# folkol/query-engines

Measured on AMD Instinct MI355X. Metric: rows/sec filter+project+group-by over 1B-row Arrow batch; % HBM roofline, higher is better.
Workload: dtype int64; 1 GPU; C4: SELECT k, SUM(a+b), COUNT(*), MIN(a), MAX(b) WHERE a > 2^19 GROUP BY k; rows_per_gpu=1000000000, groups=1024, columns=k, a, b int64 (Arrow, no nulls), parallelism=hash-sharded partial aggregate x1

## Files before the change

query-engines_amd/csrc/qe_dev.hpp:

```cpp
#ifndef QE_DEV_HPP
#define QE_DEV_HPP

#ifndef QE_OP_EQ
#define QE_OP_EQ 10
#define QE_OP_NE 11
#define QE_OP_LT 12
#define QE_OP_LE 13
#define QE_OP_GT 14
#define QE_OP_GE 15
#endif
#ifndef QE_MAX_KEYS
#define QE_MAX_KEYS 4
#define QE_MAX_AGGS 8
#define QE_MAX_COLS 8
#define QE_MAX_TERMS 8
#define QE_MAX_TOKENS 16
#endif
#ifndef QE_AGG_SUM
#define QE_AGG_SUM 1
#define QE_AGG_MIN 2
#define QE_AGG_MAX 3
#define QE_AGG_COUNT 4
#define QE_AGG_COUNT_STAR 5
#define QE_AGG_AVG 6
// ... 75 lines not shown
  qu64 cap;
  qu64* ctl;
};

struct Plan {
  DCol cols[QE_MAX_COLS];
  DTerm terms[QE_MAX_TERMS];
  DAgg aggs[QE_MAX_AGGS];
  DTable t;
  qi64 n, row_base;
  const qu32* defer_in;
  qu32* defer_out;
  qu8* ovf;
  qu64 ovf_cap;
  qi32 ncols, nterms, mask_col, naggs;
  qi32 key_mode, nkeys, key_f64, rec_bytes;
  qi32 key_col[QE_MAX_KEYS], key_shift[QE_MAX_KEYS], key_nullbit[QE_MAX_KEYS], pad0;
  qi64 key_fmask[QE_MAX_KEYS];
  qi32 lds_log2, off_cstar;
  qi32 all8;
  qi32 nn_skip;
  qi32 off_acc[QE_MAX_AGGS], off_nn[QE_MAX_AGGS], off_idx[QE_MAX_AGGS];
  qu8* part_rec;
  qi64* part_off;
  qi64 part_tw;
  qi64* part_slice;
  qi64* part_chunk;
  qi32* part_sorted;
  qi32 mp_n, mp_pass;
  qi32 part_narrow;
  qi32 lds_compact;
  qu64 mp_keep;
  qu64* host_ctl;
};

__host__ __device__ inline qi64 f64_bits(double d) { return __builtin_bit_cast(qi64, d); }
__host__ __device__ inline double bits_f64(qi64 b) { return __builtin_bit_cast(double, b); }

__host__ __device__ inline qi64 f64_okey(double d) {
  const qi64 b = f64_bits(d == 0.0 ? 0.0 : d);
  return b >= 0 ? b : (b ^ 0x7FFFFFFFFFFFFFFFll);
}
__host__ __device__ inline double okey_f64(qi64 k) { return bits_f64(k >= 0 ? k : (k ^ 0x7FFFFFFFFFFFFFFFll)); }

__host__ __device__ inline qu64 fmix64(qu64 k) {
  k ^= k >> 33;
  k *= 0xFF51AFD7ED558CCDull;
  k ^= k >> 33;
  k *= 0xC4CEB9FE1A85EC53ull;
  k ^= k >> 33;
  return k;
}

__device__ inline qu32 spill_hash(qu64 key) {
  qu32 x = (qu32)key ^ (qu32)(key >> 32) * 0x27D4EB2Fu;
  x ^= x >> 16;
  x *= 0x85EBCA6Bu;
  x ^= x >> 13;
  x *= 0xC2B2AE35u;
  return x ^ (x >> 16);
}

__device__ inline qu32 lds_hash(qu64 key) {
  const qu32 x = (qu32)key ^ (qu32)(key >> 32) * 0x85EBCA6Bu;
  return x * 0x9E3779B1u;
}
// ... 804 lines not shown
```

query-engines_amd/csrc/qe_hashagg.hip:

```cpp
#include <map>
#include <memory>
#include <mutex>

#include "qe_internal.hpp"

namespace qe {

constexpr int HA_THREADS = 512;

__device__ __forceinline__ qi64* lds_keys(char* smem) { return (qi64*)smem; }

__device__ __forceinline__ void lds_init(const Plan& P, char* smem) {
  const int SS = (1 << P.lds_log2) + 2;
  qi64* keys = lds_keys(smem);
  qu32* cst = (qu32*)(smem + P.off_cstar);
  for (int s = threadIdx.x; s < SS; s += blockDim.x) {
    keys[s] = EMPTY_KEY;
    cst[s] = 0;
  }
#pragma unroll
  for (int j = 0; j < QE_MAX_AGGS; ++j) {
    if (j >= P.naggs) break;
    const DAgg& a = P.aggs[j];
    if (a.acc != ACC_NONE) {
      qi64* acc = (qi64*)(smem + P.off_acc[j]);
      const qi64 id = acc_identity(a.acc);
      for (int s = threadIdx.x; s < SS; s += blockDim.x) acc[s] = id;
    }
    if (a.track_nn) {
      qu32* nn = (qu32*)(smem + P.off_nn[j]);
      for (int s = threadIdx.x; s < SS; s += blockDim.x) nn[s] = 0;
    }
// ... 1319 lines not shown
  int32_t lds_log2_min = 0;
  int64_t expected_groups = 0;
  int64_t create_groups = 0;
  int grid = 0;
  int64_t* part_cnt = nullptr;
  size_t part_cnt_bytes = 0;
  int64_t chunk_cap = 0;
  uint8_t* part_rec = nullptr;
  size_t part_rec_bytes = 0;
  int64_t* part_slc = nullptr;
  size_t part_slc_bytes = 0;
  bool part_wide = false;
  bool narrow_failed = false;
  bool compact_off = false;
  uint8_t* ovf = nullptr;
  uint64_t ovf_cap = 0;
  uint32_t* defer[2] = {nullptr, nullptr};
  size_t defer_words = 0;
  bool defer_dirty[2] = {false, false};
  bool ctl_rows_clean = false;
  hipEvent_t ev[2] = {nullptr, nullptr};
  double last_kernel_ms = 0.0;
  int last_launches = 0;
  int last_specialized = 0;
  uint64_t last_sig = 0;
  std::string jit_note;
  bool async = false;
  bool pending = false;
  std::unique_ptr<qe::Plan> pend_plan;
  size_t pend_lds = 0;
  int pend_out_i = 0;
  uint64_t* ctl_pin = nullptr;
  hipEvent_t ev_ctl = nullptr;
  int poisoned = 0;
  std::string poison_msg;
  qe::Keyed* keyed = nullptr;
  int32_t flags = 0;
  uint64_t version = 0;
};

namespace qe {

int hashagg_expected_groups(const qe_hashagg* h, int64_t* out) {
  QE_CHECK(h && out, QE_ERR_INVALID_ARG, "null argument");
  *out = h->create_groups;
  return QE_OK;
}

qe_ctx* hashagg_ctx(const qe_hashagg* h) { return h ? h->ctx : nullptr; }

HashaggInfo hashagg_info(const qe_hashagg* h) {
  HashaggInfo I{};
  I.ctx = h->ctx;
  I.km = h->km;
  I.rec_bytes = h->rec_bytes;
  I.naggs = h->naggs;
  I.flags = h->flags;
  for (int j = 0; j < h->naggs; ++j) I.aggs[j] = h->aggs[j];
  I.version = h->version;
  I.ctl = (uint64_t*)h->ctl;
  I.keyed = h->keyed;
  return I;
}

static AggMeta agg_meta(const qe_hashagg* h) {
  AggMeta m{};
// ... 3 lines not shown
    m.acc[j] = h->acc[j];
    m.any_x = m.any_x || h->acc[j] == ACC_SUM_X;
  }
  m.nn_implicit = h->nn_implicit;
  return m;
}

static int32_t all_nn_bits(const qe_hashagg* h) {
  if (!agg_knobs().nn_implicit) return 0;
  int32_t b = 0;
  for (int j = 0; j < h->naggs; ++j)
    if (h->aggs[j].fn != QE_AGG_COUNT_STAR) b |= 1 << j;
  return b;
}

static int nn_materialize(qe_hashagg* h, int32_t mask) {
  mask &= h->nn_implicit;
  if (!mask) return QE_OK;
  const int grid = (int)std::min<uint64_t>(div_up(h->t.cap + 2, 256), 4096);
  hipLaunchKernelGGL(k_nn_materialize, dim3(grid), dim3(256), 0, h->ctx->stream, h->t, (qi32)mask);
  QE_TRY(launch_check("k_nn_materialize"));
  h->nn_implicit &= ~mask;
  return QE_OK;
}

static size_t table_bytes(const qe_hashagg* h, uint64_t cap) {
  const uint64_t SS = cap + 2;
  size_t b = 16 * SS;
  for (int j = 0; j < h->naggs; ++j)
    b += (16 + (acc_has_idx(h->acc[j]) ? 32 : 0) + (h->acc[j] == ACC_SUM_X ? 8 * FXE_WORDS : 0)) * SS;
  return b;
}

static int table_alloc(qe_hashagg* h, uint64_t cap, void** mem, DTable* t, qu64* zero_ctl = nullptr) {
  const size_t bytes = table_bytes(h, cap);
  QE_TRY(dev_alloc(h->ctx, bytes, mem));
  const uint64_t SS = cap + 2;
  char* p = (char*)*mem;
  *t = DTable{};
  t->keys = (qi64*)p;
  p += 8 * SS;
  t->cstar = (qu64*)p;
  p += 8 * SS;
  for (int j = 0; j < h->naggs; ++j) {
    t->acc[j] = (qi64*)p;
    p += 8 * SS;
    t->nn[j] = (qu64*)p;
    p += 8 * SS;
    if (acc_has_idx(h->acc[j])) {
      t->idx[j] = (qu64*)p;
      p += 32 * SS;
    }
  }
  char* e0 = p;
  for (int j = 0; j < h->naggs; ++j)
    if (h->acc[j] == ACC_SUM_X) {
      t->ext[j] = (qu64*)p;
      p += 8 * FXE_WORDS * SS;
    }
  if (p > e0) QE_HIP(hipMemsetAsync(e0, 0, (size_t)(p - e0), h->ctx->stream));
  t->cap = cap;
  t->ctl = h->ctl;
  const int grid = (int)std::min<uint64_t>(div_up(SS, 256), 4096);
  hipLaunchKernelGGL(k_table_init, dim3(grid), dim3(256), 0, h->ctx->stream, *t, agg_meta(h), zero_ctl, 0);
  return launch_check("k_table_init");
}

static int read_ctl(qe_hashagg* h, uint64_t out[8]) {
  void* p;
  QE_TRY(ctx_pinned(h->ctx, 64, &p));
  QE_HIP(hipMemcpyAsync(p, h->ctl, 64, hipMemcpyDeviceToHost, h->ctx->stream));
  QE_TRY(ctx_sync(h->ctx));
  memcpy(out, p, 64);
  QE_CHECK((out[3] & CTL_KEY_TOO_LONG) == 0, QE_ERR_INVALID_ARG,
           "a UTF8 group key is longer than its column's max_len promised (qe_column.max_len)");
  QE_CHECK(out[3] == 0, QE_ERR_CAPACITY, "hash aggregate lost %llu groups (probe limit or overflow area)",
           (unsigned long long)out[3]);
  return QE_OK;
}

static uint64_t next_pow2(uint64_t x) {
  uint64_t p = 1;
  while (p < x) p <<= 1;
  return p;
}

static int table_grow(qe_hashagg* h, uint64_t want_cap) {
  const uint64_t cap = next_pow2(want_cap);
  if (cap <= h->t.cap) return QE_OK;
  void* mem;
  DTable nt;
  QE_TRY(table_alloc(h, cap, &mem, &nt));
  QE_HIP(hipMemsetAsync(h->ctl, 0, 8, h->ctx->stream));
  const int grid = (int)std::min<uint64_t>(div_up(h->t.cap + 2, 256), 8192);
  hipLaunchKernelGGL(k_rehash, dim3(grid), dim3(256), 0, h->ctx->stream, h->t, nt, agg_meta(h));
  QE_TRY(launch_check("k_rehash"));
  uint64_t c[8];
  QE_TRY(read_ctl(h, c));
  QE_CHECK(c[3] == 0, QE_ERR_CAPACITY, "hash table rehash lost %llu groups", (unsigned long long)c[3]);
  dev_free(h->ctx, h->table_mem);
  h->table_mem = mem;
  h->t = nt;
  return QE_OK;
}

static int import_records(qe_hashagg* h, const void* recs, int64_t nrec) {
  if (nrec <= 0) return QE_OK;
  const int grid = (int)std::min<uint64_t>(div_up((uint64_t)nrec, 256), 8192);
  hipLaunchKernelGGL(k_import, dim3(grid), dim3(256), 0, h->ctx->stream, (const uint8_t*)recs, nrec, h->rec_bytes,
                     h->t, agg_meta(h));
  QE_TRY(launch_check("k_import"));
  uint64_t c[8];
  QE_TRY(read_ctl(h, c));
  QE_CHECK(c[3] == 0, QE_ERR_CAPACITY, "hash table import lost %llu groups", (unsigned long long)c[3]);
  return QE_OK;
}

static int ensure_defer(qe_hashagg* h, int64_t n) {
  const size_t words = (size_t)div_up((uint64_t)n, 32);
  if (words <= h->defer_words) return QE_OK;
  for (int i = 0; i < 2; ++i) {
    dev_free(h->ctx, h->defer[i]);
// ... 331 lines not shown
  QE_TRY(jit_launch(ctx, fc, (int)G.g, P));
  QE_TRY(launch_check("qe_pcount"));
  QE_TRY(exclusive_scan_i64(ctx, cnt, off, (int64_t)G.cells));
  void* pin;
  QE_TRY(ctx_pinned(ctx, 8, &pin));
  QE_HIP(hipMemcpyAsync(pin, off + G.cells, 8, hipMemcpyDeviceToHost, ctx->stream));
  QE_TRY(ctx_sync(ctx));
  const int64_t R = *(int64_t*)pin;
  QE_TRY(ensure_overflow(h, PART_OVF_RECORDS));
  P.ovf = h->ovf;
  P.ovf_cap = h->ovf_cap;
  if (R > 0) {
    QE_TRY(grow_buffer(&h->part_rec, &h->part_rec_bytes, (size_t)R * rb, ctx, "partition records"));
    P.part_off = (qi64*)off;
    P.part_rec = h->part_rec;
    QE_TRY(jit_launch(ctx, fs, (int)G.g, P, sblock));
    QE_TRY(launch_check("qe_pscatter"));
  }
  const CountedSlices S = counted_slices(R, G.np, ctx->num_cus);
  QE_TRY(grow_buffer(&h->part_slc, &h->part_slc_bytes, S.slice_bytes, ctx, "partition slices"));
  hipLaunchKernelGGL(k_part_slices, dim3(1), dim3(1024), 0, ctx->stream, (const qi64*)off, (qi32)G.np, (qi64)G.g,
                     (qi64)S.cw, (qi64*)h->part_slc);
  QE_TRY(launch_check("k_part_slices"));
  P.n = R;
  P.part_tw = S.cw;
  P.part_rec = h->part_rec;
  P.part_slice = (qi64*)h->part_slc;
  *grid = (int)S.max_slices;
  h->jit_note = "radix-partitioned: " + std::to_string(G.np) + " buckets, " + std::to_string(R) + " records of " +
                std::to_string(rb) + " B (" + record_words_note(L) + (staged ? ", staged scatter" : "");
  return QE_OK;
}

static int launch_pass(qe_hashagg* h, Plan& P, size_t& lds, hipFunction_t pfn, int pgrid, int pass, int mp,
                       int out_i, const uint32_t* defer_in, int pblock = 0) {
  qe_ctx* ctx = h->ctx;
  const int64_t n = P.n;
  QE_CHECK(pass < 64, QE_ERR_CAPACITY, "hash aggregate did not converge after %d passes", pass);
  if (h->defer_dirty[out_i]) {
    QE_HIP(hipMemsetAsync(h->defer[out_i], 0, h->defer_words * 4, ctx->stream));
    h->defer_dirty[out_i] = false;
  }
  if (!h->ctl_rows_clean) QE_HIP(hipMemsetAsync(h->ctl + 1, 0, 16, ctx->stream));
  h->ctl_rows_clean = false;
  int32_t tracked = 0;
  for (int j = 0; j < P.naggs; ++j)
    if (P.aggs[j].track_nn) tracked |= 1 << j;
  QE_TRY(nn_materialize(h, tracked));
  P.nn_skip = h->nn_implicit;
  P.t = h->t;
  P.defer_in = defer_in;
  P.defer_out = h->defer[out_i];
  const int64_t waves = (int64_t)div_up((uint64_t)n, 256);
  const int per_cu = lds ? std::max<int>(1, std::min<int>(8, (int)((160 * 1024) / lds))) : 8;
  const int64_t gcap = std::min<int64_t>((int64_t)ctx->num_cus * per_cu, h->grid);
  int grid = (int)std::min<int64_t>((int64_t)div_up((uint64_t)waves, HA_THREADS / 64), gcap);
  if (grid < 1) grid = 1;
  hipFunction_t jfn = pfn;
  int jgrid = pgrid;
  if (pfn) {
  } else if (lds && ctx->jit) {
    static std::mutex memo_mu;
    static std::map<std::string, std::pair<hipFunction_t, int>> memo;
    const std::string key = plan_shape_key(ctx, P);
    int bpc = 0;
    bool have = false;
// ... 23 lines not shown
        h->jit_note.clear();
        if (P.lds_compact) h->jit_note = "compact LDS table: " + std::to_string(P.lds_compact) + " slots";
      } else {
        h->jit_note = qe_last_error();
        jfn = nullptr;
      }
    } else {
      h->jit_note = "plan shape not specialisable";
    }
  } else if (h->jit_note.rfind("partitioning unavailable", 0) != 0) {
    h->jit_note = lds ? "jit disabled" : "global-only launch";
  }
  bool own_layout = false;
  for (int j = 0; j < h->naggs; ++j) own_layout = own_layout || h->acc[j] == ACC_SUM_X || P.aggs[j].share;
  if (!jfn && lds && (lds > HA_LDS_BUDGET || (own_layout && ctx->jit))) {
    size_t b = 0;
    int log2 = P.lds_log2;
    while (log2 >= h->lds_log2_min && (b = lds_layout_at(h, &P, log2, true)) > HA_LDS_BUDGET) --log2;
    if (log2 < h->lds_log2_min || log2 < 8) {
      P.lds_log2 = 0;
      lds = 0;
    } else {
      lds = b;
    }
    const int pc = lds ? std::max<int>(1, std::min<int>(8, (int)((160 * 1024) / lds))) : 8;
    grid = (int)std::max<int64_t>(1, std::min<int64_t>((int64_t)div_up((uint64_t)waves, HA_THREADS / 64),
                                                       std::min<int64_t>((int64_t)ctx->num_cus * pc, h->grid)));
  }
  if (!jfn) {
    const int pcu = lds ? std::max<int>(1, std::min<int>(2048 / HA_THREADS, (int)((160 * 1024) / lds))) : 2048 / HA_THREADS;
    h->jit_note += std::string(h->jit_note.empty() ? "" : "; ") + "generic kernel: " + std::to_string(lds / 1024) +
                   " KiB LDS table, " + std::to_string(pcu) + " workgroups per CU";
  }
  if (pass > 0 || mp > 0) QE_HIP(hipEventRecord(h->ev[0], ctx->stream));
  if (jfn) {
    QE_TRY(jit_launch(ctx, jfn, jgrid, P, pfn ? (pblock ? pblock : pagg_block()) : fused_block(P.lds_log2)));
  } else {
    QE_TRY(launch_hashagg(P, grid, lds, ctx->stream));
  }
  h->last_specialized = jfn ? 1 : 0;
  {
    const uint64_t k = jfn ? jit_kernel_signature(jfn) : 0x6E65726963ull;
    const uint64_t shape = jfn ? ((uint64_t)jgrid << 20) ^ (uint64_t)(pfn ? (pblock ? pblock : pagg_block()) : fused_block(P.lds_log2))
                               : ((uint64_t)grid << 20) ^ (uint64_t)lds;
    h->last_sig = fmix64(k ^ fmix64(shape));
  }
  QE_TRY(launch_check("k_hashagg"));
  QE_HIP(hipEventRecord(h->ev[1], ctx->stream));
  QE_HIP(hipMemcpyAsync(h->ctl_pin, h->ctl, 64, hipMemcpyDeviceToHost, ctx->stream));
  QE_HIP(hipEventRecord(h->ev_ctl, ctx->stream));
  return QE_OK;
}

static int settle_pass(qe_hashagg* h, const Plan& P, int* out_i, const uint32_t** defer_in, bool* done) {
  uint64_t c[8];
  QE_HIP(hipEventSynchronize(h->ev_ctl));
  memcpy(c, h->ctl_pin, 64);
  QE_CHECK((c[3] & CTL_KEY_TOO_LONG) == 0, QE_ERR_INVALID_ARG,
           "a UTF8 group key is longer than its column's max_len promised (qe_column.max_len)");
  QE_CHECK(c[3] == 0, QE_ERR_CAPACITY, "hash aggregate lost %llu groups (probe limit or overflow area)",
           (unsigned long long)c[3]);
  {
    float ms = 0.f;
    QE_HIP(hipEventElapsedTime(&ms, h->ev[0], h->ev[1]));
    h->last_kernel_ms += ms;
    h->last_launches += 1;
  }
  QE_CHECK(c[3] == 0, QE_ERR_CAPACITY, "hash aggregate lost %llu groups (overflow area)", (unsigned long long)c[3]);
  h->narrow_failed = P.part_narrow && (c[7] & 1) != 0;
  if (P.lds_compact && (c[7] & 2)) h->compact_off = true;
  const uint64_t groups = c[0], deferred = c[1], ovf_recs = std::min<uint64_t>(c[2], P.ovf_cap);
  h->ctl_rows_clean = c[1] == 0 && c[2] == 0;
  *done = true;
  if (deferred == 0 && ovf_recs == 0) {
    if (groups * 2 > h->t.cap) QE_TRY(table_grow(h, 4 * h->t.cap));
    h->known_groups = (int64_t)groups;
    return QE_OK;
  }
  QE_TRY(table_grow(h, std::max<uint64_t>(4 * h->t.cap, 2 * (groups + ovf_recs))));
  if (ovf_recs) QE_TRY(import_records(h, h->ovf, (int64_t)ovf_recs));
  if (deferred == 0) return QE_OK;
  h->defer_dirty[*out_i] = true;
  *defer_in = h->defer[*out_i];
  *out_i ^= 1;
  *done = false;
  return QE_OK;
}

static void adapt_after_update(qe_hashagg* h, size_t lds, int lds_log2) {
  if (h->known_groups > 0 && h->ctx->jit) {
    if (lds && h->known_groups * 5 / 4 > ((int64_t)1 << lds_log2)) h->lds_log2 = 0;
    if (h->lds_log2 == 0) h->expected_groups = std::max<int64_t>(h->expected_groups, h->known_groups);
  }
}

static int settle_body(qe_hashagg* h) {
  Plan& P = *h->pend_plan;
  int out_i = h->pend_out_i;
  const uint32_t* defer_in = nullptr;
// ... 155 lines not shown
  if (c.path != PATH_COMPACT_SPILL) {
    P = T;
    *lds = jl;
    *mp_n = c.mp_n;
    *taken = !spill;
  }
  if (spill) {
    Plan& X = c.path == PATH_SPILL ? P : T;
    QE_TRY(spill_update(h, X, jl, rows, K, finished));
    if (*finished) {
      h->row_base += rows;
      adapt_after_update(h, jl, X.lds_log2);
    } else if (c.path == PATH_SPILL) {
      *taken = true;
    }
  }
  return QE_OK;
}

static int run_update(qe_hashagg* h, Plan& P) {
  qe_ctx* ctx = h->ctx;
  QE_TRY(settle_pending(h));
  const int64_t rows = P.n;
  if (rows == 0) return QE_OK;
  size_t lds = lds_layout(h, &P);
  P.mp_n = 0;
  P.mp_pass = 0;
  P.ovf = h->ovf;
  P.ovf_cap = h->ovf_cap;
  QE_TRY(ensure_defer(h, rows));
  h->known_groups = -1;
  h->last_kernel_ms = 0.0;
  h->last_launches = 0;
  h->chunk_cap = 0;
  hipFunction_t pfn = nullptr;
  int pgrid = 0;
  QE_HIP(hipEventRecord(h->ev[0], ctx->stream));
  const AggKnobs K = lds ? agg_knobs() : agg_knobs_now();
  AggLadderIn in;
  in.jit = ctx->jit != 0;
  in.num_cus = ctx->num_cus;
  in.expected_groups = h->expected_groups;
  in.compact_off = h->compact_off;
  in.regular_bytes = lds;
  Plan S;
  if (!lds) {
    S = P;
    in.compact_ok = in.jit && compact_ok(P);
    in.compact_slot_bytes = in.compact_ok ? compact_slot_bytes(P) : 0;
    in.fused_budget = lds_budget(ctx);
    in.pagg_budget = pagg_lds_budget(pagg_block());
  }
  const AggLadder ladder = agg_ladder(in, K, [&](int log2) { return lds_layout_at(h, &S, log2); });
  int mp_n = 0, rung = 0;
  for (bool taken = false; !taken; ++rung) {
    bool finished = false;
    QE_TRY(try_rung(h, P, ladder.c[rung], rows, K, &lds, &mp_n, &taken, &finished));
    if (finished) return QE_OK;
  }
  const AggCandidate& path = ladder.c[rung - 1];
  const Plan P_rows = P;
  for (;;) {
  if (path.path == PATH_PARTITION) {
    Plan Q = P;
    if (partition_rows(h, Q, path.tlog2, K, &pfn, &pgrid) == QE_OK) {
      P = Q;
// ... 9 lines not shown
        return QE_OK;
      }
    } else {
      h->jit_note = std::string("partitioning unavailable: ") + qe_last_error();
      pfn = nullptr;
    }
  }
  int out_i = 0;
  for (int mp = 0; mp < std::max(1, mp_n); ++mp) {
    P.mp_pass = mp;
    const uint32_t* defer_in = nullptr;
    for (int pass = 0;; ++pass) {
      QE_TRY(launch_pass(h, P, lds, pfn, pgrid, pass, mp, out_i, defer_in));
      if (h->async && pass == 0 && mp_n == 0 && !pfn) {
        if (!h->pend_plan) h->pend_plan.reset(new Plan());
        *h->pend_plan = P;
        h->pend_lds = lds;
        h->pend_out_i = out_i;
        h->pending = true;
        h->row_base += rows;
        return QE_OK;
      }
      bool done = false;
      QE_TRY(settle_pass(h, P, &out_i, &defer_in, &done));
      if (done) break;
    }
  }
  if (pfn && h->narrow_failed) {
    h->narrow_failed = false;
    h->part_wide = true;
    h->chunk_cap = 0;
    P = P_rows;
    pfn = nullptr;
    QE_HIP(hipEventRecord(h->ev[0], ctx->stream));
    continue;
  }
  break;
  }
  if (mp_n)
    h->jit_note = "multi-pass: " + std::to_string(mp_n) + " bucket passes" + (P.lds_compact ? " (compact table)" : "") +
                  (h->last_specialized ? "" : "; " + h->jit_note);
  h->row_base += rows;
  adapt_after_update(h, lds, P.lds_log2);
  return QE_OK;
}

}

extern "C" {

int qe_hashagg_create(qe_ctx* ctx, int32_t nkeys, const int32_t* key_types, int32_t naggs, const qe_agg_desc* aggs,
                      int64_t expected_groups, qe_hashagg** out) {
  return qe_hashagg_create_ex(ctx, nkeys, key_types, naggs, aggs, expected_groups, 0, out);
}

int qe_hashagg_create_ex(qe_ctx* ctx, int32_t nkeys, const int32_t* key_types, int32_t naggs, const qe_agg_desc* aggs,
                         int64_t expected_groups, int32_t flags, qe_hashagg** out) {
  QE_TRY(ctx_enter(ctx));
  QE_CHECK((flags & ~(QE_HASHAGG_DETERMINISTIC | QE_HASHAGG_FAST_FP64)) == 0, QE_ERR_INVALID_ARG, "unknown flags 0x%x",
           flags);
  QE_CHECK((flags & QE_HASHAGG_DETERMINISTIC) == 0 || (flags & QE_HASHAGG_FAST_FP64) == 0, QE_ERR_INVALID_ARG,
           "QE_HASHAGG_DETERMINISTIC and QE_HASHAGG_FAST_FP64 exclude each other");
  const bool det = (flags & QE_HASHAGG_FAST_FP64) == 0;
  QE_CHECK(out, QE_ERR_INVALID_ARG, "null out");
  QE_CHECK(nkeys >= 0 && nkeys <= QE_MAX_KEYS, QE_ERR_UNSUPPORTED, "0..%d group keys supported", QE_MAX_KEYS);
  QE_CHECK(naggs >= 0 && naggs <= QE_MAX_AGGS, QE_ERR_UNSUPPORTED, "0..%d aggregates supported", QE_MAX_AGGS);
  QE_CHECK(nkeys == 0 || key_types, QE_ERR_INVALID_ARG, "null key_types");
  QE_CHECK(naggs == 0 || aggs, QE_ERR_INVALID_ARG, "null aggs");
  qe_hashagg* h = new qe_hashagg();
  h->ctx = ctx;
  h->naggs = naggs;
  h->flags = flags;
  auto bail = [&](int code) {
    for (hipEvent_t e : {h->ev[0], h->ev[1], h->ev_ctl})
      if (e) (void)hipEventDestroy(e);
    if (h->ctl_pin) pinned_slot_free(h->ctl_pin, h->ctx->stream);
    if (h->keyed) keyed_destroy(ctx, h->keyed);
    delete h;
    return code;
  };
  int32_t dev_types[QE_MAX_KEYS] = {};
  {
    int32_t dn = 0;
    const int st = keyed_create(ctx, nkeys, key_types, expected_groups > 0 ? expected_groups : 1024, &h->keyed, &dn,
                                dev_types);
    if (st != QE_OK) return bail(st);
    nkeys = dn;
    key_types = dev_types;
  }
  h->nkeys = nkeys;
  if (nkeys == 0) {
    h->km.mode = 0;
  } else if (nkeys == 1 && (key_types[0] == QE_TYPE_INT64 || key_types[0] == QE_TYPE_FLOAT64)) {
    h->km.mode = 1;
  } else {
    h->km.mode = 2;
    int bit = 0;
    for (int k = 0; k < nkeys; ++k) {
      int w;
      switch (key_types[k]) {
        case QE_TYPE_INT32:
        case QE_TYPE_DATE32: w = 32; break;
        case QE_TYPE_UINT8: w = 8; break;
        default:
          return bail(fail(QE_ERR_UNSUPPORTED,
                           "group key %d: type %d cannot be packed (multi-key groups take uint8/int32/date32)", k,
                           key_types[k]));
      }
      h->km.shift[k] = bit;
// ... 3 lines not shown
      bit += 1;
    }
    if (bit > 63) return bail(fail(QE_ERR_UNSUPPORTED, "group keys need %d bits (max 63)", bit));
  }
  h->km.nkeys = nkeys;
  for (int k = 0; k < nkeys; ++k) {
    h->key_types[k] = key_types[k];
    h->km.type[k] = key_types[k];
  }
  h->rec_bytes = 24;
  for (int j = 0; j < naggs; ++j) {
    const qe_agg_desc& d = aggs[j];
    h->aggs[j] = d;
    const bool f = d.input_type == QE_TYPE_FLOAT64;
    const bool i = d.input_type == QE_TYPE_INT64 || d.input_type == QE_TYPE_INT32 ||
                   d.input_type == QE_TYPE_DATE32 || d.input_type == QE_TYPE_UINT8;
    if (d.fn != QE_AGG_COUNT_STAR && d.fn != QE_AGG_COUNT && !i && !f)
      return bail(fail(QE_ERR_UNSUPPORTED, "aggregate %d: input type %d (int64/int32/date32/uint8/fp64 only)", j,
                       d.input_type));
    switch (d.fn) {
      case QE_AGG_SUM: h->acc[j] = f ? (det ? ACC_SUM_X : ACC_SUM_F) : ACC_SUM_I; break;
      case QE_AGG_MIN: h->acc[j] = f ? ACC_MIN_F : ACC_MIN_I; break;
      case QE_AGG_MAX: h->acc[j] = f ? ACC_MAX_F : ACC_MAX_I; break;
      case QE_AGG_AVG: h->acc[j] = det ? ACC_SUM_X : ACC_SUM_F; break;
      case QE_AGG_COUNT:
      case QE_AGG_COUNT_STAR: h->acc[j] = ACC_NONE; break;
      default: return bail(fail(QE_ERR_UNSUPPORTED, "aggregate %d: unknown function %d", j, d.fn));
    }
    h->rec_bytes += agg_rec_bytes(h->acc[j]);
  }
  if (hipEventCreate(&h->ev[0]) != hipSuccess || hipEventCreate(&h->ev[1]) != hipSuccess ||
      hipEventCreateWithFlags(&h->ev_ctl, hipEventDisableTiming) != hipSuccess)
    return bail(fail(QE_ERR_DEVICE, "hipEventCreate failed"));
  if (pinned_slot_alloc(&h->ctl_pin) != QE_OK) return bail(QE_ERR_OOM);
  if (dev_alloc(ctx, 64, (void**)&h->ctl) != QE_OK) return bail(fail(QE_ERR_OOM, "control allocation failed"));
  const int64_t eg = expected_groups > 0 ? expected_groups : 1024;
  h->expected_groups = eg;
  h->create_groups = eg;
  const LdsRange lr = lds_table_range(eg, h->acc, naggs, !ctx->jit, lds_budget(ctx));
  h->lds_log2 = lr.log2;
  h->lds_log2_min = lr.log2_min;
  const int per_cu = h->lds_log2 ? std::max<int>(1, std::min<int>(8, (int)((160 * 1024) / lds_bytes_min(h->acc, naggs, h->lds_log2, !ctx->jit)))) : 8;
  h->grid = ctx->num_cus * per_cu;
  if (h->lds_log2) {
    h->ovf_cap = (uint64_t)h->grid * (((uint64_t)1 << h->lds_log2) + 2);
    if (dev_alloc(ctx, h->ovf_cap * h->rec_bytes, (void**)&h->ovf) != QE_OK) {
      dev_free(ctx, h->ctl);
      return bail(fail(QE_ERR_OOM, "overflow area allocation failed"));
    }
  }
  const int st = table_alloc(h, std::max<uint64_t>(1024, next_pow2((uint64_t)(2 * eg))), &h->table_mem, &h->t, h->ctl);
  h->nn_implicit = all_nn_bits(h);
  if (st != QE_OK) {
    dev_free(ctx, h->ovf);
    dev_free(ctx, h->ctl);
    return bail(st);
  }
  h->ctl_rows_clean = true;
  *out = h;
  return QE_OK;
}

int qe_hashagg_destroy(qe_hashagg* h) {
  if (!h) return QE_OK;
  (void)hipSetDevice(h->ctx->device);
  qe_ctx* ctx = h->ctx;
  void* bufs[] = {h->table_mem, h->ctl, h->ovf, h->part_cnt, h->part_rec, h->part_slc, h->defer[0], h->defer[1]};
  for (void* b : bufs) dev_free(ctx, b);
  if (h->keyed) keyed_destroy(ctx, h->keyed);
  for (int i = 0; i < 2; ++i) {
    if (h->ev[i]) (void)hipEventDestroy(h->ev[i]);
  }
  if (h->ev_ctl) (void)hipEventDestroy(h->ev_ctl);
  pinned_slot_free(h->ctl_pin, ctx->stream);
  delete h;
  return QE_OK;
}

int qe_hashagg_last_kernel_kind(qe_hashagg* h, int32_t* specialized, char* note, int32_t note_len) {
  QE_CHECK(h && specialized, QE_ERR_INVALID_ARG, "null argument");
  *specialized = h->last_specialized;
  if (note && note_len > 0) {
    strncpy(note, h->jit_note.c_str(), (size_t)note_len - 1);
    note[note_len - 1] = 0;
  }
  return QE_OK;
}

int qe_hashagg_last_kernel_signature(qe_hashagg* h, uint64_t* sig) {
  QE_CHECK(h && sig, QE_ERR_INVALID_ARG, "null argument");
  *sig = h->last_sig;
  return QE_OK;
}

int qe_hashagg_last_kernel_time(qe_hashagg* h, double* ms, int32_t* launches) {
  QE_CHECK(h && ms, QE_ERR_INVALID_ARG, "null argument");
  QE_TRY(ctx_enter(h->ctx));
  QE_TRY(settle_pending(h));
  *ms = h->last_kernel_ms;
  if (launches) *launches = h->last_launches;
  return QE_OK;
}

int qe_hashagg_last_chunk_stats(qe_hashagg* h, int64_t* chunks, int64_t* full_chunks, int64_t* records) {
  QE_CHECK(h && chunks && full_chunks && records, QE_ERR_INVALID_ARG, "null argument");
  QE_TRY(ctx_enter(h->ctx));
  QE_TRY(settle_pending(h));
  *chunks = *full_chunks = *records = 0;
  if (h->chunk_cap <= 0 || !h->part_cnt) return QE_OK;
  QE_TRY(ctx_sync(h->ctx));
  int64_t ids = 0;
  QE_HIP(hipMemcpy(&ids, h->part_cnt, 8, hipMemcpyDeviceToHost));
  ids = std::max<int64_t>(0, std::min<int64_t>(ids, h->chunk_cap));
  std::vector<int64_t> meta((size_t)ids);
  if (ids) QE_HIP(hipMemcpy(meta.data(), h->part_cnt + 1, (size_t)ids * 8, hipMemcpyDeviceToHost));
  for (const int64_t w : meta) {
    if (w < 0) continue;
    const int64_t fill = w & 0xFFFFFFFFll;
    *chunks += 1;
    *full_chunks += fill == PART_CH ? 1 : 0;
    *records += fill;
  }
  return QE_OK;
}

int qe_hashagg_set_async(qe_hashagg* h, int32_t enable) {
  QE_CHECK(h, QE_ERR_INVALID_ARG, "null state");
  QE_TRY(ctx_enter(h->ctx));
  if (!enable) QE_TRY(settle_pending(h));
  h->async = enable != 0;
  return QE_OK;
}

int qe_hashagg_reset(qe_hashagg* h) {
  QE_CHECK(h, QE_ERR_INVALID_ARG, "null state");
  QE_TRY(ctx_enter(h->ctx));
  if (h->pending) {
    h->pending = false;
    h->defer_dirty[h->pend_out_i] = true;
  }
  h->poisoned = 0;
  h->poison_msg.clear();
  const int grid = (int)std::min<uint64_t>(div_up(h->t.cap + 2, 256), 4096);
  hipLaunchKernelGGL(k_table_init, dim3(grid), dim3(256), 0, h->ctx->stream, h->t, agg_meta(h), (qu64*)h->ctl, 1);
  QE_TRY(launch_check("k_table_init"));
  h->nn_implicit = all_nn_bits(h);
  h->ctl_rows_clean = true;
  h->row_base = 0;
  h->known_groups = 0;
  ++h->version;
  return QE_OK;
}

int qe_hashagg_set_row_base(qe_hashagg* h, int64_t row_base) {
  QE_CHECK(h && row_base >= 0, QE_ERR_INVALID_ARG, "bad arguments");
  h->row_base = row_base;
  return QE_OK;
}

static_assert(sizeof(Plan) <= 4096, "kernel argument must stay under 4 KiB");

int qe_hashagg_update_fused(qe_hashagg* h, const qe_column* cols, int32_t ncols, const qe_fused_spec* spec) {
  QE_CHECK(h && cols && spec, QE_ERR_INVALID_ARG, "null argument");
  QE_TRY(ctx_enter(h->ctx));
  if (keyed_dict(h->keyed)) return keyed_update_fused(h, cols, ncols, spec);
  return hashagg_update_fused_raw(h, cols, ncols, spec);
}

int qe_hashagg_update(qe_hashagg* h, const qe_column* keys, const qe_column* agg_inputs, const qe_column* mask) {
  QE_CHECK(h, QE_ERR_INVALID_ARG, "null state");
  QE_TRY(ctx_enter(h->ctx));
  QE_CHECK(h->nkeys == 0 || keys, QE_ERR_INVALID_ARG, "null keys");
  if (keyed_dict(h->keyed)) return keyed_update(h, keys, agg_inputs, mask);
  return hashagg_update_raw(h, keys, agg_inputs, mask);
}

}

// ... 306 lines not shown
```

query-engines_amd/csrc/qe_jit.hip:

```cpp
#include <hip/hiprtc.h>
#include <stdio.h>
#include <stdlib.h>
#include <fcntl.h>
#include <string.h>
#include <sys/stat.h>
#include <unistd.h>

#include <map>
#include <mutex>
#include <sstream>
#include <vector>

#include "qe_internal.hpp"

namespace qe {

static const char* kDevHeader =
#include "qe_dev.inc"
    ;

namespace {

struct Expr {
  std::string v;
// ... 782 lines not shown
      << "            qi64 w[" << L.words << "];\n";
    emit_record_words(P, L, ex, "w", o);
    emit_fit_check(L, "w", o);
    const char* wt = L.narrow ? "qi32" : "qi64";
    o << "            " << wt << "* const dst = (" << wt << "*)(P.part_rec + pos * " << RB << "ull);\n";
    for (int q = 0; q < L.words; ++q) o << "            dst[" << q << "] = (" << wt << ")w[" << q << "];\n";
    o << "          }\n          kb += (qu32)__popcll(bal[r]);\n        }\n"
      << "        sp_cid[b] = nid;\n        sp_fill[b] = tot - room;\n"
      << "      }\n    }\n"
      << "    if (act == 0) continue;\n";
  } else if (P.mp_n > 1)
    o << "#pragma unroll\n    for (int r = 0; r < 4; ++r)\n"
      << "      if (((act >> r) & 1) && (P.mp_pass < 0 ? spill_hash((qu64)key[r]) < P.mp_keep\n"
      << "                                              : (qu32)__umul64hi(fmix64((qu64)key[r]), (qu64)P.mp_n) != (qu32)P.mp_pass))\n"
      << "        act &= ~(1u << r);\n"
      << "    if (act == 0) continue;\n";
  if (compact)
    emit_agg_rows_c(P, o, val, ok, "P.row_base + r0 + 128 * (r >> 1) + (r & 1)", "r0 + 128 * (r >> 1) + (r & 1)");
  else
    emit_agg_rows(P, o, val, ok, "P.row_base + r0 + 128 * (r >> 1) + (r & 1)", "r0 + 128 * (r >> 1) + (r & 1)", fxq,
                  log2 <= 8);
  o << (pf ? "    } while (0);\n  }\n  }\n" : "  }\n");
  if (fxq) {
    o << "  if (q_n) {\n";
    emit_fx_queue_run(P, o, "q_n");
    o << "  }\n";
  }
  if (spill)
    o << "#pragma unroll\n  for (int b = 0; b < SB; ++b)\n"
      << "    if ((threadIdx.x & 63) == 0 && sp_cid[b] >= 0) P.part_chunk[1 + sp_cid[b]] = ((qi64)b << 32) | (qi64)sp_fill[b];\n"
      << "  if (nfit) atomicOr(&P.t.ctl[7], 1ull);\n";
  if (compact) emit_flush_c(P, o);
  else emit_flush(P, o);
  o << "  __syncthreads();\n  if (threadIdx.x == 0 && s_newg) atomicAdd(&P.t.ctl[0], (qu64)s_newg);\n}\n";
  static const bool fx_inline = [] {
    const char* e = getenv("QE_FX_INLINE");
    return !(e && e[0] == '0');
  }();
  *src = std::string(fx_inline ? "#define QE_FX_INLINE 1\n" : "") + kDevHeader + o.str();
  return true;
}

PartLayout part_layout(const Plan& P) {
  PartLayout L{};
  bool knull = false, vnull = false, cnull = false;
  for (int k = 0; k < P.nkeys; ++k) knull = knull || P.cols[P.key_col[k]].valid != nullptr;
  int nv = 0;
  unsigned cm = 0;
  for (int j = 0; j < P.naggs; ++j) {
    if (P.aggs[j].pkind == 0) continue;
    ++nv;
    vnull = vnull || P.aggs[j].track_nn;
    L.row = L.row || acc_is_f64mm(P.aggs[j].acc);
    for (int t = 0; t < P.aggs[j].ntok; ++t)
      if (P.aggs[j].tok[t].op == T_COL) cm |= 1u << P.aggs[j].tok[t].arg;
  }
  for (int c = 0; c < P.ncols; ++c)
    if ((cm >> c) & 1u) cnull = cnull || P.cols[c].valid != nullptr;
  const int wv = 1 + nv + ((knull || vnull) ? 1 : 0);
  const int wc = 1 + __builtin_popcount(cm) + ((knull || cnull) ? 1 : 0);
  L.colmode = wc < wv;
  int w = 1;
  for (int j = 0; j < P.naggs; ++j) L.val_word[j] = (!L.colmode && P.aggs[j].pkind != 0) ? w++ : -1;
  for (int c = 0; c < QE_MAX_COLS; ++c) L.col_word[c] = (L.colmode && ((cm >> c) & 1u)) ? w++ : -1;
  L.flags_word = (knull || (L.colmode ? cnull : vnull)) ? w++ : -1;
  L.row_word = L.row ? w++ : -1;
  L.words = w;
// ... 969 lines not shown
bool selproj_nt(const Plan& P) {
  const char* e = getenv("QE_SELPROJ_NT");
  if (e && *e) return e[0] == '1';
  return P.n > (64ll << 20);
}

std::string plan_shape_key(const qe_ctx* ctx, const Plan& P) {
  Plan k;
  memset(&k, 0, sizeof k);
  memcpy(&k, &P, sizeof P);
  for (int c = 0; c < QE_MAX_COLS; ++c) {
    k.cols[c].p = (const void*)(uintptr_t)(P.cols[c].p != nullptr);
    k.cols[c].valid = (const qu8*)(uintptr_t)(P.cols[c].valid != nullptr);
  }
  for (int t = 0; t < QE_MAX_TERMS; ++t) k.terms[t].lit = 0;
  for (int j = 0; j < QE_MAX_AGGS; ++j) {
    k.aggs[j].rhs_lit = 0;
    for (int t = 0; t < QE_MAX_TOKENS; ++t) k.aggs[j].tok[t].lit = 0;
  }
  memset(&k.t, 0, sizeof k.t);
  k.n = k.row_base = 0;
  k.defer_in = nullptr;
  k.defer_out = nullptr;
  k.ovf = nullptr;
  k.ovf_cap = 0;
  k.part_rec = nullptr;
  k.part_off = nullptr;
  k.part_tw = 0;
  k.part_slice = nullptr;
  k.part_chunk = nullptr;
  k.part_sorted = nullptr;
  k.mp_keep = 0;
  k.host_ctl = nullptr;
  const int32_t extra[2] = {ctx->device, use_nt() ? 1 : 0};
  return std::string((const char*)&k, sizeof k) + std::string((const char*)extra, sizeof extra);
}

int selproj_block(int mode) {
  static const int all = [] {
    const char* e = getenv("QE_SELPROJ_BLOCK");
    const int b = e && *e ? atoi(e) : 0;
    return (b == 256 || b == 512 || b == 1024) ? b : 0;
  }();
  static const int lb = [] {
    const char* e = getenv("QE_SELPROJ_LB_BLOCK");
    const int b = e && *e ? atoi(e) : 1024;
    return (b == 256 || b == 512) ? b : 1024;
  }();
  if (all) return all;
  return (mode == SP_PERSIST || mode == SP_COUNTER) ? lb : 256;
}

int selproj_lbw() {
  static const int v = [] {
    const char* e = getenv("QE_SELPROJ_LBW");
    const int k = e && *e ? atoi(e) : 1;
    return (k == 2 || k == 4) ? k : 1;
  }();
  return v;
}

constexpr size_t kSelprojStageBytes = 128 * 1024;

int selproj_rows_per_thread(const Plan& P, int mode) {
  static const int env = [] {
    const char* e = getenv("QE_SELPROJ_ROWS");
// ... 738 lines not shown
```

Measured before the change: 274.4 billion rows/s.

## Publish counters from last block to pinned memory and double-buffer small hash tables

The fused JIT kernel now has its last-finishing block, found with an atomic ticket, copy the control counters into pinned host memory and set a sequence flag. The host spin-waits on that flag instead of issuing a D2H memcpy and an event synchronize, and resolves kernel timing lazily. Resetting a small table now swaps in a pre-cleared spare table, and the spare is re-initialised after the next launch, taking the table-init kernel off the critical path. This costs extra memory, a host busy-wait loop and extra atomics at kernel end.

```diff
diff --git a/query-engines_amd/csrc/qe_dev.hpp b/query-engines_amd/csrc/qe_dev.hpp
--- a/query-engines_amd/csrc/qe_dev.hpp
+++ b/query-engines_amd/csrc/qe_dev.hpp
@@ -131,6 +131,9 @@
   qi32 lds_compact;
   qu64 mp_keep;
   qu64* host_ctl;
+  qu64* pub;
+  qu64* pub_flag;
+  qu64 pub_seq;
 };
 
 __host__ __device__ inline qi64 f64_bits(double d) { return __builtin_bit_cast(qi64, d); }
diff --git a/query-engines_amd/csrc/qe_hashagg.hip b/query-engines_amd/csrc/qe_hashagg.hip
--- a/query-engines_amd/csrc/qe_hashagg.hip
+++ b/query-engines_amd/csrc/qe_hashagg.hip
@@ -1,3 +1,5 @@
+#include <atomic>
+#include <chrono>
 #include <map>
 #include <memory>
 #include <mutex>
@@ -1383,6 +1385,14 @@
   int pend_out_i = 0;
   uint64_t* ctl_pin = nullptr;
   hipEvent_t ev_ctl = nullptr;
+  uint64_t* pub_flag = nullptr;
+  uint64_t pub_seq = 0;
+  bool published = false;
+  bool time_pending = false;
+  void* spare_mem = nullptr;
+  DTable spare_t{};
+  qu64* spare_ctl = nullptr;
+  bool spare_clean = false;
   int poisoned = 0;
   std::string poison_msg;
   qe::Keyed* keyed = nullptr;
@@ -1452,7 +1462,8 @@
   return b;
 }
 
-static int table_alloc(qe_hashagg* h, uint64_t cap, void** mem, DTable* t, qu64* zero_ctl = nullptr) {
+static int table_alloc(qe_hashagg* h, uint64_t cap, void** mem, DTable* t, qu64* zero_ctl = nullptr,
+                       qu64* ctl = nullptr) {
   const size_t bytes = table_bytes(h, cap);
   QE_TRY(dev_alloc(h->ctx, bytes, mem));
   const uint64_t SS = cap + 2;
@@ -1480,7 +1491,7 @@
     }
   if (p > e0) QE_HIP(hipMemsetAsync(e0, 0, (size_t)(p - e0), h->ctx->stream));
   t->cap = cap;
-  t->ctl = h->ctl;
+  t->ctl = ctl ? ctl : h->ctl;
   const int grid = (int)std::min<uint64_t>(div_up(SS, 256), 4096);
   hipLaunchKernelGGL(k_table_init, dim3(grid), dim3(256), 0, h->ctx->stream, *t, agg_meta(h), zero_ctl, 0);
   return launch_check("k_table_init");
@@ -1505,9 +1516,49 @@
   return p;
 }
 
+static bool table_small(const DTable& t) { return t.cap + 2 <= (uint64_t)FS_THREADS * FS_PER; }
+
+static void spare_drop(qe_hashagg* h) {
+  dev_free(h->ctx, h->spare_mem);
+  h->spare_mem = nullptr;
+  h->spare_t = DTable{};
+  h->spare_clean = false;
+}
+
+static int spare_clear(qe_hashagg* h) {
+  if (!h->spare_mem || h->spare_clean) return QE_OK;
+  const int grid = (int)std::min<uint64_t>(div_up(h->spare_t.cap + 2, 256), 4096);
+  hipLaunchKernelGGL(k_table_init, dim3(grid), dim3(256), 0, h->ctx->stream, h->spare_t, agg_meta(h), h->spare_ctl, 1);
+  QE_TRY(launch_check("k_table_init"));
+  h->spare_clean = true;
+  return QE_OK;
+}
+
+static int spare_swap_in(qe_hashagg* h, bool* swapped) {
+  *swapped = false;
+  if (!table_small(h->t)) return QE_OK;
+  if (h->spare_mem && h->spare_t.cap != h->t.cap) spare_drop(h);
+  if (!h->spare_mem) {
+    if (!h->spare_ctl) QE_TRY(dev_alloc(h->ctx, 64, (void**)&h->spare_ctl));
+    if (table_alloc(h, h->t.cap, &h->spare_mem, &h->spare_t, h->spare_ctl, h->spare_ctl) != QE_OK) {
+      spare_drop(h);
+      return QE_OK;
+    }
+    h->spare_clean = true;
+  }
+  if (!h->spare_clean) return QE_OK;
+  std::swap(h->table_mem, h->spare_mem);
+  std::swap(h->t, h->spare_t);
+  std::swap(h->ctl, h->spare_ctl);
+  h->spare_clean = false;
+  *swapped = true;
+  return QE_OK;
+}
+
 static int table_grow(qe_hashagg* h, uint64_t want_cap) {
   const uint64_t cap = next_pow2(want_cap);
   if (cap <= h->t.cap) return QE_OK;
+  spare_drop(h);
   void* mem;
   DTable nt;
   QE_TRY(table_alloc(h, cap, &mem, &nt));
@@ -1905,6 +1956,8 @@
   return QE_OK;
 }
 
+static int resolve_kernel_time(qe_hashagg* h);
+
 static int launch_pass(qe_hashagg* h, Plan& P, size_t& lds, hipFunction_t pfn, int pgrid, int pass, int mp,
                        int out_i, const uint32_t* defer_in, int pblock = 0) {
   qe_ctx* ctx = h->ctx;
@@ -1994,7 +2047,12 @@
     h->jit_note += std::string(h->jit_note.empty() ? "" : "; ") + "generic kernel: " + std::to_string(lds / 1024) +
                    " KiB LDS table, " + std::to_string(pcu) + " workgroups per CU";
   }
+  QE_TRY(resolve_kernel_time(h));
   if (pass > 0 || mp > 0) QE_HIP(hipEventRecord(h->ev[0], ctx->stream));
+  h->published = jfn && !pfn && P.mp_n <= 1;
+  P.pub = h->published ? (qu64*)h->ctl_pin : nullptr;
+  P.pub_flag = h->published ? (qu64*)h->pub_flag : nullptr;
+  P.pub_seq = h->published ? ++h->pub_seq : 0;
   if (jfn) {
     QE_TRY(jit_launch(ctx, jfn, jgrid, P, pfn ? (pblock ? pblock : pagg_block()) : fused_block(P.lds_log2)));
   } else {
@@ -2009,24 +2067,57 @@
   }
   QE_TRY(launch_check("k_hashagg"));
   QE_HIP(hipEventRecord(h->ev[1], ctx->stream));
-  QE_HIP(hipMemcpyAsync(h->ctl_pin, h->ctl, 64, hipMemcpyDeviceToHost, ctx->stream));
+  if (!h->published) QE_HIP(hipMemcpyAsync(h->ctl_pin, h->ctl, 64, hipMemcpyDeviceToHost, ctx->stream));
   QE_HIP(hipEventRecord(h->ev_ctl, ctx->stream));
+  QE_TRY(spare_clear(h));
+  return QE_OK;
+}
+
+static int resolve_kernel_time(qe_hashagg* h) {
+  if (!h->time_pending) return QE_OK;
+  h->time_pending = false;
+  float ms = 0.f;
+  QE_HIP(hipEventSynchronize(h->ev[1]));
+  QE_HIP(hipEventElapsedTime(&ms, h->ev[0], h->ev[1]));
+  h->last_kernel_ms += ms;
+  return QE_OK;
+}
+
+static int wait_published(qe_hashagg* h) {
+  volatile uint64_t* pf = h->pub_flag;
+  auto t0 = std::chrono::steady_clock::now();
+  for (uint32_t i = 1; *pf != h->pub_seq; ++i) {
+    if ((i & 1023) != 0) continue;
+    if (std::chrono::steady_clock::now() - t0 < std::chrono::microseconds(50)) continue;
+    t0 = std::chrono::steady_clock::now();
+    const hipError_t e = hipEventQuery(h->ev_ctl);
+    if (e == hipSuccess) {
+      if (*pf != h->pub_seq) return fail(QE_ERR_DEVICE, "hash aggregate kernel finished without publishing its counters");
+      break;
+    }
+    if (e != hipErrorNotReady) return fail(QE_ERR_DEVICE, "hash aggregate kernel failed: %s", hipGetErrorString(e));
+    (void)hipGetLastError();
+  }
+  std::atomic_thread_fence(std::memory_order_acquire);
   return QE_OK;
 }
 
 static int settle_pass(qe_hashagg* h, const Plan& P, int* out_i, const uint32_t** defer_in, bool* done) {
   uint64_t c[8];
-  QE_HIP(hipEventSynchronize(h->ev_ctl));
+  if (h->published) QE_TRY(wait_published(h));
+  else QE_HIP(hipEventSynchronize(h->ev_ctl));
   memcpy(c, h->ctl_pin, 64);
   QE_CHECK((c[3] & CTL_KEY_TOO_LONG) == 0, QE_ERR_INVALID_ARG,
            "a UTF8 group key is longer than its column's max_len promised (qe_column.max_len)");
   QE_CHECK(c[3] == 0, QE_ERR_CAPACITY, "hash aggregate lost %llu groups (probe limit or overflow area)",
            (unsigned long long)c[3]);
-  {
+  h->last_launches += 1;
+  if (h->published) {
+    h->time_pending = true;
+  } else {
     float ms = 0.f;
     QE_HIP(hipEventElapsedTime(&ms, h->ev[0], h->ev[1]));
     h->last_kernel_ms += ms;
-    h->last_launches += 1;
   }
   QE_CHECK(c[3] == 0, QE_ERR_CAPACITY, "hash aggregate lost %llu groups (overflow area)", (unsigned long long)c[3]);
   h->narrow_failed = P.part_narrow && (c[7] & 1) != 0;
@@ -2248,6 +2339,7 @@
   h->known_groups = -1;
   h->last_kernel_ms = 0.0;
   h->last_launches = 0;
+  h->time_pending = false;
   h->chunk_cap = 0;
   hipFunction_t pfn = nullptr;
   int pgrid = 0;
@@ -2323,6 +2415,7 @@
     h->chunk_cap = 0;
     P = P_rows;
     pfn = nullptr;
+    QE_TRY(resolve_kernel_time(h));
     QE_HIP(hipEventRecord(h->ev[0], ctx->stream));
     continue;
   }
@@ -2366,6 +2459,7 @@
     for (hipEvent_t e : {h->ev[0], h->ev[1], h->ev_ctl})
       if (e) (void)hipEventDestroy(e);
     if (h->ctl_pin) pinned_slot_free(h->ctl_pin, h->ctx->stream);
+    if (h->pub_flag) pinned_slot_free(h->pub_flag, h->ctx->stream);
     if (h->keyed) keyed_destroy(ctx, h->keyed);
     delete h;
     return code;
@@ -2435,7 +2529,8 @@
   if (hipEventCreate(&h->ev[0]) != hipSuccess || hipEventCreate(&h->ev[1]) != hipSuccess ||
       hipEventCreateWithFlags(&h->ev_ctl, hipEventDisableTiming) != hipSuccess)
     return bail(fail(QE_ERR_DEVICE, "hipEventCreate failed"));
-  if (pinned_slot_alloc(&h->ctl_pin) != QE_OK) return bail(QE_ERR_OOM);
+  if (pinned_slot_alloc(&h->ctl_pin) != QE_OK || pinned_slot_alloc(&h->pub_flag) != QE_OK) return bail(QE_ERR_OOM);
+  h->pub_flag[0] = 0;
   if (dev_alloc(ctx, 64, (void**)&h->ctl) != QE_OK) return bail(fail(QE_ERR_OOM, "control allocation failed"));
   const int64_t eg = expected_groups > 0 ? expected_groups : 1024;
   h->expected_groups = eg;
@@ -2468,7 +2563,8 @@
   if (!h) return QE_OK;
   (void)hipSetDevice(h->ctx->device);
   qe_ctx* ctx = h->ctx;
-  void* bufs[] = {h->table_mem, h->ctl, h->ovf, h->part_cnt, h->part_rec, h->part_slc, h->defer[0], h->defer[1]};
+  void* bufs[] = {h->table_mem, h->ctl,         h->spare_mem, h->spare_ctl, h->ovf,
+                  h->part_cnt,  h->part_rec,    h->part_slc,  h->defer[0],  h->defer[1]};
   for (void* b : bufs) dev_free(ctx, b);
   if (h->keyed) keyed_destroy(ctx, h->keyed);
   for (int i = 0; i < 2; ++i) {
@@ -2476,6 +2572,7 @@
   }
   if (h->ev_ctl) (void)hipEventDestroy(h->ev_ctl);
   pinned_slot_free(h->ctl_pin, ctx->stream);
+  pinned_slot_free(h->pub_flag, ctx->stream);
   delete h;
   return QE_OK;
 }
@@ -2500,6 +2597,7 @@
   QE_CHECK(h && ms, QE_ERR_INVALID_ARG, "null argument");
   QE_TRY(ctx_enter(h->ctx));
   QE_TRY(settle_pending(h));
+  QE_TRY(resolve_kernel_time(h));
   *ms = h->last_kernel_ms;
   if (launches) *launches = h->last_launches;
   return QE_OK;
@@ -2544,9 +2642,13 @@
   }
   h->poisoned = 0;
   h->poison_msg.clear();
-  const int grid = (int)std::min<uint64_t>(div_up(h->t.cap + 2, 256), 4096);
-  hipLaunchKernelGGL(k_table_init, dim3(grid), dim3(256), 0, h->ctx->stream, h->t, agg_meta(h), (qu64*)h->ctl, 1);
-  QE_TRY(launch_check("k_table_init"));
+  bool swapped = false;
+  QE_TRY(spare_swap_in(h, &swapped));
+  if (!swapped) {
+    const int grid = (int)std::min<uint64_t>(div_up(h->t.cap + 2, 256), 4096);
+    hipLaunchKernelGGL(k_table_init, dim3(grid), dim3(256), 0, h->ctx->stream, h->t, agg_meta(h), (qu64*)h->ctl, 1);
+    QE_TRY(launch_check("k_table_init"));
+  }
   h->nn_implicit = all_nn_bits(h);
   h->ctl_rows_clean = true;
   h->row_base = 0;
diff --git a/query-engines_amd/csrc/qe_jit.hip b/query-engines_amd/csrc/qe_jit.hip
--- a/query-engines_amd/csrc/qe_jit.hip
+++ b/query-engines_amd/csrc/qe_jit.hip
@@ -838,7 +838,21 @@
       << "  if (nfit) atomicOr(&P.t.ctl[7], 1ull);\n";
   if (compact) emit_flush_c(P, o);
   else emit_flush(P, o);
-  o << "  __syncthreads();\n  if (threadIdx.x == 0 && s_newg) atomicAdd(&P.t.ctl[0], (qu64)s_newg);\n}\n";
+  const bool publish = !spill && P.mp_n <= 1;
+  if (publish) o << "  __builtin_amdgcn_s_waitcnt(0x0F70);\n";
+  o << "  __syncthreads();\n  if (threadIdx.x == 0 && s_newg) atomicAdd(&P.t.ctl[0], (qu64)s_newg);\n";
+  if (publish)
+    o << "  if (threadIdx.x == 0 && P.pub_seq) {\n"
+      << "    const qu64 ticket = __hip_atomic_fetch_add(&P.t.ctl[6], 1ull, __ATOMIC_RELEASE, __HIP_MEMORY_SCOPE_AGENT);\n"
+      << "    if (ticket == (qu64)gridDim.x - 1) {\n"
+      << "      __threadfence();\n"
+      << "      __hip_atomic_store(&P.t.ctl[6], 0ull, __ATOMIC_RELAXED, __HIP_MEMORY_SCOPE_AGENT);\n"
+      << "      qu64 cw[8];\n"
+      << "#pragma unroll\n      for (int w = 0; w < 8; ++w) cw[w] = __hip_atomic_load(&P.t.ctl[w], __ATOMIC_RELAXED, __HIP_MEMORY_SCOPE_AGENT);\n"
+      << "#pragma unroll\n      for (int w = 0; w < 8; ++w) __hip_atomic_store(&P.pub[w], cw[w], __ATOMIC_RELAXED, __HIP_MEMORY_SCOPE_SYSTEM);\n"
+      << "      __hip_atomic_store(P.pub_flag, P.pub_seq, __ATOMIC_RELEASE, __HIP_MEMORY_SCOPE_SYSTEM);\n"
+      << "    }\n  }\n";
+  o << "}\n";
   static const bool fx_inline = [] {
     const char* e = getenv("QE_FX_INLINE");
     return !(e && e[0] == '0');
@@ -1874,6 +1888,9 @@
   k.part_sorted = nullptr;
   k.mp_keep = 0;
   k.host_ctl = nullptr;
+  k.pub = nullptr;
+  k.pub_flag = nullptr;
+  k.pub_seq = 0;
   const int32_t extra[2] = {ctx->device, use_nt() ? 1 : 0};
   return std::string((const char*)&k, sizeof k) + std::string((const char*)extra, sizeof extra);
 }
```

After: 274.0 billion rows/s. About the same (-0.1%).
